# mightypirate1/DRL-Tetris

Measured on AMD Instinct MI355X. Metric: env-steps/sec at 64k parallel 20x10 boards, higher is better.
Workload: dtype u32

## Files before the change

drl-tetris_amd/csrc/tetris_engine.h:

```cpp
#pragma once
#include "tetris_layout.h"
#include "tetris_tables.h"

#if defined(__clang__)
#define TE_UNROLL _Pragma("unroll")
#else
#define TE_UNROLL _Pragma("GCC unroll 8")
#endif

namespace te {

TE_HD int ctz32(uint32_t v) { return __builtin_ctz(v); }
TE_HD int clz32(uint32_t v) { return __builtin_clz(v); }
#if defined(__HIP_DEVICE_COMPILE__)
TE_HD uint32_t ld_stream(const uint32_t* p) { return __builtin_nontemporal_load(p); }
TE_HD void st_stream(uint32_t* p, uint32_t v) { __builtin_nontemporal_store(v, p); }
#else
TE_HD uint32_t ld_stream(const uint32_t* p) { return *p; }
TE_HD void st_stream(uint32_t* p, uint32_t v) { *p = v; }
#endif

#if defined(TE_PATH_COUNTERS) && !defined(__HIPCC__)
enum PathCounter { PC_KICK = 0, PC_KICK_2ND, PC_KICK_3RD, PC_KICK_FAILED, PC_KICK_DOWN, PC_DROP_EXACT, PC_RT_OFF_SPAWN,
                   PC_GARBAGE_ROW, PC_GARBAGE_LIFT2, PC_DEATH_GARBAGE, PC_DEATH_SPAWN, PC_TIMER_LOCK, PC_KEY_KICK, PC_KEY_KICK_FAILED,
// ... 5 lines not shown
#endif

enum MemMode : int { MEM_STREAM = 0, MEM_AGENT = 1, MEM_AFFINE = 2 };
#if defined(__HIP_DEVICE_COMPILE__)
TE_HD uint32_t ld_agent(const uint32_t* p) { return __hip_atomic_load(p, __ATOMIC_RELAXED, __HIP_MEMORY_SCOPE_AGENT); }
TE_HD void st_agent(uint32_t* p, uint32_t v) { __hip_atomic_store(p, v, __ATOMIC_RELAXED, __HIP_MEMORY_SCOPE_AGENT); }
#else
TE_HD uint32_t ld_agent(const uint32_t* p) { return *p; }
TE_HD void st_agent(uint32_t* p, uint32_t v) { *p = v; }
#endif
#if defined(__HIP_DEVICE_COMPILE__)
TE_HD __amdgpu_buffer_rsrc_t te_rsrc(const void* base) {
    return __builtin_amdgcn_make_buffer_rsrc(const_cast<void*>(base), (short)0, -1, 0x00020000);
}
constexpr int TE_AUX_NT = 2, TE_AUX_SC1 = 16;
TE_HD uint32_t ldw_b(const uint32_t* base, uint32_t o, size_t row_bytes, int mem = MEM_STREAM) {
    const __amdgpu_buffer_rsrc_t r = te_rsrc(base);
    if (mem == MEM_AGENT || mem == MEM_AFFINE) return __builtin_amdgcn_raw_buffer_load_b32(r, (int)o, (int)(uint32_t)row_bytes, TE_AUX_SC1);
    return __builtin_amdgcn_raw_buffer_load_b32(r, (int)o, (int)(uint32_t)row_bytes, TE_AUX_NT);
}
TE_HD void stw_b(uint32_t* base, uint32_t o, size_t row_bytes, uint32_t v, int mem = MEM_STREAM) {
    const __amdgpu_buffer_rsrc_t r = te_rsrc(base);
    if (mem == MEM_AGENT) __builtin_amdgcn_raw_buffer_store_b32(v, r, (int)o, (int)(uint32_t)row_bytes, TE_AUX_SC1);
    else if (mem == MEM_AFFINE) __builtin_amdgcn_raw_buffer_store_b32(v, r, (int)o, (int)(uint32_t)row_bytes, 0);
    else __builtin_amdgcn_raw_buffer_store_b32(v, r, (int)o, (int)(uint32_t)row_bytes, TE_AUX_NT);
}
#else
TE_HD uint32_t ldw_b(const uint32_t* base, uint32_t o, size_t row_bytes, int mem = MEM_STREAM) {
    const uint32_t* p = (const uint32_t*)((const char*)base + row_bytes + o);
    return mem != MEM_STREAM ? ld_agent(p) : ld_stream(p);
}
TE_HD void stw_b(uint32_t* base, uint32_t o, size_t row_bytes, uint32_t v, int mem = MEM_STREAM) {
    uint32_t* p = (uint32_t*)((char*)base + row_bytes + o);
    if (mem != MEM_STREAM) st_agent(p, v); else st_stream(p, v);
}
#endif
TE_HD uint32_t ldw(const uint32_t* base, uint32_t o, size_t word_off, int mem = MEM_STREAM) { return ldw_b(base, o, word_off * 4u, mem); }
TE_HD void stw(uint32_t* base, uint32_t o, size_t word_off, uint32_t v, int mem = MEM_STREAM) { stw_b(base, o, word_off * 4u, v, mem); }
struct RowStride { size_t ws; };
template <int N>
struct RowTable { uint32_t bytes[N]; };
TE_HD size_t row_bytes(const RowStride& r, int w) { return (size_t)w * r.ws * 4u; }
template <int N>
TE_HD size_t row_bytes(const RowTable<N>& r, int w) { return r.bytes[w]; }
#if defined(__HIP_DEVICE_COMPILE__)
TE_HD void add_word(uint32_t* p, uint32_t v) { (void)__hip_atomic_fetch_add(p, v, __ATOMIC_RELAXED, __HIP_MEMORY_SCOPE_AGENT); }
#else
TE_HD void add_word(uint32_t* p, uint32_t v) { *p += v; }
#endif
#if defined(__HIP_DEVICE_COMPILE__)
TE_HD uint32_t mul24(uint32_t a, uint32_t b) { return __umul24(a, b); }
#else
TE_HD uint32_t mul24(uint32_t a, uint32_t b) { return a * b; }
#endif
TE_HD int imin(int a, int b) { return a < b ? a : b; }
TE_HD int imax(int a, int b) { return a > b ? a : b; }
TE_HD uint32_t f2u(float f) { union { float f; uint32_t u; } v; v.f = f; return v.u; }
TE_HD float u2f(uint32_t u) { union { float f; uint32_t u; } v; v.u = u; return v.f; }

// ... 86 lines not shown
template <int P>
struct Game {
    Player pl[P];
    uint32_t seed16;
    int round_over, last_winner;
    uint32_t flags;
    uint32_t episode;
    uint32_t steps;
    uint32_t add_lines, add_sent;
    uint32_t status;
    uint32_t draw0, draw1;
};

template <class ROWS>
TE_HD void load_player_rows(const uint32_t* s, uint32_t o, const ROWS& rows, Player& q, bool tint, bool queue = true, int mem = MEM_STREAM) {
    for (int c = 0; c < NCOL; c++) q.col[c] = ldw_b(s, o, row_bytes(rows, W_COL0 + c), mem);
    if (tint)
        for (int k = 0; k < 3; k++)
            for (int c = 0; c < NCOL; c++) q.tint[k][c] = ldw_b(s, o, row_bytes(rows, W_TINT0 + 10 * k + c), mem);
    uint32_t w = ldw_b(s, o, row_bytes(rows, W_PIECE), mem);
    q.kind = w & 7; q.rot = (w >> 3) & 3; q.x = (int)((w >> 5) & 15) - 4; q.y = (w >> 9) & 31;
    q.next = (w >> 14) & 7; q.dead = (w >> 17) & 1; q.lock_armed = (w >> 18) & 1; q.reward = (w >> 19) & 255;
    w = ldw_b(s, o, row_bytes(rows, W_MISC), mem);
    q.inc_count = w & 255; q.combo_count = (w >> 8) & 255; q.line_count = (w >> 16) & 255;
    q.qlen = (w >> 24) & 15; q.q_overflow = (w >> 28) & 3;
    if (!queue) { q.inc_count = 0; q.qlen = 0; q.q_overflow = 0; }
    q.time_ms = (int32_t)ldw_b(s, o, row_bytes(rows, W_TIME), mem);
    w = ldw_b(s, o, row_bytes(rows, W_DROPCOMBO), mem);
    q.drop_delay = w & 0xFFFF; q.combo_remaining = w >> 16;
    q.drop_time = (int32_t)ldw_b(s, o, row_bytes(rows, W_DROP_TIME), mem);
    q.speedup_time = (int32_t)ldw_b(s, o, row_bytes(rows, W_SPEEDUP_TIME), mem);
    q.lock_time = (int32_t)ldw_b(s, o, row_bytes(rows, W_LOCK_TIME), mem);
    q.combo_start = (int32_t)ldw_b(s, o, row_bytes(rows, W_COMBO_START), mem);
    q.combo_time = (int32_t)ldw_b(s, o, row_bytes(rows, W_COMBO_TIME), mem);
    q.incoming = queue ? u2f(ldw_b(s, o, row_bytes(rows, W_INCOMING), mem)) : 0.0f;
    q.min_remaining = queue ? (int32_t)ldw_b(s, o, row_bytes(rows, W_MIN_REMAINING), mem) : 1000;
    q.piece_draws = ldw_b(s, o, row_bytes(rows, W_PIECE_DRAWS), mem);
    q.hole_draws = queue ? ldw_b(s, o, row_bytes(rows, W_HOLE_DRAWS), mem) : 0u;
    q.pgroup = ldw_b(s, o, row_bytes(rows, W_PIECE_GROUP), mem);
    w = ldw_b(s, o, row_bytes(rows, W_STATS0), mem); q.lines_sent = w & 0xFFFF; q.lines_cleared = w >> 16;
    w = ldw_b(s, o, row_bytes(rows, W_STATS1), mem); q.lines_blocked = w & 0xFFFF; q.max_combo = w >> 16;
    w = ldw_b(s, o, row_bytes(rows, W_STATS2), mem); q.lines_seen = w & 0xFFFF; q.garbage_cleared = w >> 16;
    q.q_loaded = queue && q.qlen > 0;
    q.pf_ok = 0; q.pf_raw.lo = 0; q.pf_raw.hi = 0;
    if (queue)
        for (int i = 0; i < FIFO_CAP; i++) { q.qcount[i] = 0; q.qdelay[i] = 0; }
    if (q.q_loaded) {
        for (int i = 0; i < FIFO_CAP / 2; i++) {
            uint32_t cw = ldw_b(s, o, row_bytes(rows, W_FIFO_COUNT0 + i), mem);
            q.qcount[2 * i] = (int16_t)(cw & 0xFFFF);
            q.qcount[2 * i + 1] = (int16_t)(cw >> 16);
        }
        for (int i = 0; i < FIFO_CAP; i++) q.qdelay[i] = (int32_t)ldw_b(s, o, row_bytes(rows, W_FIFO_DELAY0 + i), mem);
    }
}

TE_HD void load_player(const uint32_t* s, uint32_t o, size_t ws, Player& q, bool tint, bool queue = true, int mem = MEM_STREAM) {
    load_player_rows(s, o, RowStride{ws}, q, tint, queue, mem);
}

template <int P, class ROWS>
TE_HD void load_game_words_rows(const Ref& gr, const ROWS& rows, Game<P>& g, bool counters = false, int mem = MEM_STREAM) {
    uint32_t meta = ldw_b(gr.s, gr.o, row_bytes(rows, G_META), mem);
    g.seed16 = meta & 0xFFFFu;
    g.round_over = (meta >> 16) & 1;
    g.last_winner = (int)((meta >> 17) & 0xF) - 1;
    g.flags = (meta >> 21) & 7u;
    g.episode = ldw_b(gr.s, gr.o, row_bytes(rows, G_EPISODE), mem);
    g.steps = counters ? ldw_b(gr.s, gr.o, row_bytes(rows, G_STEPS), mem) : 0u;
    g.add_lines = 0; g.add_sent = 0;
    g.status = 0;
}

template <int P>
TE_HD void load_game_words(const Ref& gr, Game<P>& g, bool counters = false, int mem = MEM_STREAM) {
    load_game_words_rows<P>(gr, RowStride{gr.ws}, g, counters, mem);
}

template <int P, class ROWS, class GROWS>
TE_HD void load_game_rows(const Geo& geo_in, size_t slot, const ROWS& rows, const GROWS& grows, Game<P>& g, bool tint = false, bool queue = true,
                          bool counters = false, int mem = MEM_STREAM) {
    Geo geo = geo_in;
    geo.P = P;
    load_game_words_rows<P>(game_ref(geo, slot), grows, g, counters, mem);
    TE_UNROLL
    for (int p = 0; p < P; p++) {
        const Ref r = board_ref(geo, p, slot);
        load_player_rows(r.s, r.o, rows, g.pl[p], tint, queue, mem);
    }
}
template <int P>
TE_HD void load_game(const Geo& geo_in, size_t slot, Game<P>& g, bool tint = false, bool queue = true, bool counters = false, int mem = MEM_STREAM) {
    load_game_rows<P>(geo_in, slot, RowStride{(size_t)P * geo_in.stride}, RowStride{geo_in.stride}, g, tint, queue, counters, mem);
}

template <class ROWS>
TE_HD void store_player_rows(uint32_t* s, uint32_t o, const ROWS& rows, const Player& q, bool tint, bool queue = true, int mem = MEM_STREAM) {
    for (int c = 0; c < NCOL; c++) stw_b(s, o, row_bytes(rows, W_COL0 + c), q.col[c], mem);
    if (tint)
        for (int k = 0; k < 3; k++)
            for (int c = 0; c < NCOL; c++) stw_b(s, o, row_bytes(rows, W_TINT0 + 10 * k + c), q.tint[k][c], mem);
    stw_b(s, o, row_bytes(rows, W_PIECE), (uint32_t)q.kind | ((uint32_t)q.rot << 3) | ((uint32_t)(q.x + 4) << 5) | ((uint32_t)q.y << 9) |
                              ((uint32_t)q.next << 14) | ((uint32_t)q.dead << 17) | ((uint32_t)q.lock_armed << 18) |
                              ((uint32_t)(q.reward & 255) << 19), mem);
    stw_b(s, o, row_bytes(rows, W_MISC), (uint32_t)(q.inc_count & 255) | ((uint32_t)(q.combo_count & 255) << 8) |
                             ((uint32_t)(q.line_count & 255) << 16) | ((uint32_t)q.qlen << 24) | ((uint32_t)q.q_overflow << 28), mem);
    stw_b(s, o, row_bytes(rows, W_TIME), (uint32_t)q.time_ms, mem);
    stw_b(s, o, row_bytes(rows, W_DROPCOMBO), ((uint32_t)q.drop_delay & 0xFFFF) | (q.combo_remaining << 16), mem);
    stw_b(s, o, row_bytes(rows, W_DROP_TIME), (uint32_t)q.drop_time, mem);
    stw_b(s, o, row_bytes(rows, W_SPEEDUP_TIME), (uint32_t)q.speedup_time, mem);
    stw_b(s, o, row_bytes(rows, W_LOCK_TIME), (uint32_t)q.lock_time, mem);
    stw_b(s, o, row_bytes(rows, W_COMBO_START), (uint32_t)q.combo_start, mem);
    stw_b(s, o, row_bytes(rows, W_COMBO_TIME), (uint32_t)q.combo_time, mem);
    if (queue) stw_b(s, o, row_bytes(rows, W_INCOMING), f2u(q.incoming), mem);
    stw_b(s, o, row_bytes(rows, W_MIN_REMAINING), (uint32_t)q.min_remaining, mem);
    stw_b(s, o, row_bytes(rows, W_PIECE_DRAWS), q.piece_draws, mem);
    if (queue) stw_b(s, o, row_bytes(rows, W_HOLE_DRAWS), q.hole_draws, mem);
    stw_b(s, o, row_bytes(rows, W_PIECE_GROUP), q.pgroup, mem);
    stw_b(s, o, row_bytes(rows, W_STATS0), (q.lines_sent & 0xFFFF) | (q.lines_cleared << 16), mem);
    stw_b(s, o, row_bytes(rows, W_STATS1), (q.lines_blocked & 0xFFFF) | (q.max_combo << 16), mem);
    stw_b(s, o, row_bytes(rows, W_STATS2), (q.lines_seen & 0xFFFF) | (q.garbage_cleared << 16), mem);
    if (queue && (q.q_loaded || q.qlen > 0)) {
        for (int i = 0; i < FIFO_CAP / 2; i++)
            stw_b(s, o, row_bytes(rows, W_FIFO_COUNT0 + i), ((uint32_t)q.qcount[2 * i] & 0xFFFF) | ((uint32_t)q.qcount[2 * i + 1] << 16), mem);
        for (int i = 0; i < FIFO_CAP; i++) stw_b(s, o, row_bytes(rows, W_FIFO_DELAY0 + i), (uint32_t)q.qdelay[i], mem);
    }
}

TE_HD void store_player(uint32_t* s, uint32_t o, size_t ws, const Player& q, bool tint, bool queue = true, int mem = MEM_STREAM) {
    store_player_rows(s, o, RowStride{ws}, q, tint, queue, mem);
}

template <int P, class ROWS>
TE_HD void store_game_words_rows(const Ref& gr, const ROWS& rows, const Game<P>& g, bool counters = false, int mem = MEM_STREAM) {
    stw_b(gr.s, gr.o, row_bytes(rows, G_META), g.seed16 | ((uint32_t)g.round_over << 16) | ((uint32_t)(g.last_winner + 1) << 17) | (g.flags << 21), mem);
    stw_b(gr.s, gr.o, row_bytes(rows, G_EPISODE), g.episode, mem);
    if (counters) stw_b(gr.s, gr.o, row_bytes(rows, G_STEPS), g.steps, mem);
    if (g.add_lines) add_word((uint32_t*)((char*)gr.s + row_bytes(rows, G_LINES) + gr.o), g.add_lines);
    if (g.add_sent) add_word((uint32_t*)((char*)gr.s + row_bytes(rows, G_SENT) + gr.o), g.add_sent);
}

template <int P>
TE_HD void store_game_words(const Ref& gr, const Game<P>& g, bool counters = false, int mem = MEM_STREAM) {
    store_game_words_rows<P>(gr, RowStride{gr.ws}, g, counters, mem);
}

template <int P, class ROWS, class GROWS>
TE_HD void store_game_rows(const Geo& geo_in, size_t slot, const ROWS& rows, const GROWS& grows, const Game<P>& g, bool tint = false, bool queue = true,
                           bool counters = false, int mem = MEM_STREAM) {
    Geo geo = geo_in;
    geo.P = P;
    store_game_words_rows<P>(game_ref(geo, slot), grows, g, counters, mem);
// ... 236 lines not shown
TE_HD int combo_expire(const Ctx& cx, Player& q, int32_t t) {
    int32_t left = q.combo_start + q.combo_time - t;
    q.combo_remaining = left < 0 ? 0u : ((uint32_t)left & 0xFFFFu);
    if (t > q.combo_start + q.combo_time && q.combo_count != 0) {
        float duration = 1.f + (float)t / 60000.f * 0.1f;
        double v = cx.combo_pow[q.combo_count] * (double)duration;
        int lines = (int)((uint32_t)(int64_t)v & 0xFFFFu);
        q.combo_count = 0;
        q.line_count = 0;
        return lines;
    }
    return 0;
}


TE_HD bool spawn_next(const Ctx& cx, Player& q, uint32_t seed16, uint32_t& status) {
    q.kind = q.next;
    q.rot = spawn_rot(q.kind);
    q.x = (NCOL - 4) / 2;
    q.y = 0;
    if (q.piece_draws + cx.margin >= cx.n_draws) {
        status |= ST_NEED_EXTEND;
        if (q.piece_draws >= cx.n_draws) status |= ST_STREAM_EXHAUSTED;
    }
    q.next = (int)((q.pgroup >> (4u * (q.piece_draws & 7u))) & 7u);
    q.piece_draws++;
    if ((q.piece_draws & 7u) == 0u) {
        q.pgroup = pack_group(q.pf_ok ? q.pf_raw : table_group_raw(cx, seed16, q.piece_draws, status));
        q.pf_ok = 0;
    }
    uint32_t shape = shape_of(cx, q.kind, q.rot);
    if (!fits_spawn_col(cx, q, shape, 0)) { stamp(cx, q, shape); TE_COUNT(PC_DEATH_SPAWN); return true; }
    return false;
}

TE_HD int score_clears(const Ctx& cx, Player& q, int cleared) {
    q.lines_cleared = (q.lines_cleared + (uint32_t)cleared) & 0xFFFFu;
    if (cleared == 0) { q.combo_time -= 200; return 0; }
    int amount = cx.queue ? q_block(q, cleared - 1, q.time_ms, true) : cleared - 1;
    q.lines_sent = (q.lines_sent + (uint32_t)amount) & 0xFFFFu;
    combo_gain(q, q.time_ms, cleared);
    return amount;
}

TE_HD void lock_piece(const Ctx& cx, Player& q) {
    uint32_t shape = shape_of(cx, q.kind, q.rot);
    q.y += drop_distance(cx, q, shape);
    stamp(cx, q, shape);
    q.drop_time = q.time_ms;
    q.lock_armed = 0;
}

TE_HD int settle(const Ctx& cx, Player& q, uint32_t seed16, uint32_t& status) {
    int sent = score_clears(cx, q, clear_rows(cx, q));
    if (spawn_next(cx, q, seed16, status)) return -1;
    return sent;
}

TE_HD bool soft_drop(const Ctx& cx, Player& q) {
    const uint32_t shape = shape_of(cx, q.kind, q.rot);
    if (q.x == (NCOL - 4) / 2 ? fits_spawn_col(cx, q, shape, q.y + 1) : fits_at(cx, q, shape, q.x, q.y + 1)) {
        q.y++;
        q.drop_time = q.time_ms;
        q.lock_armed = 0;
        return true;
    }
    if (!q.lock_armed) q.lock_time = q.time_ms + 400;
    q.lock_armed = 1;
    return false;
}
// ... 15 lines not shown
    q.hole_draws++;
    uint32_t bottom = 1u << (cx.H - 1);
    for (int c = 0; c < NCOL; c++) q.col[c] = (q.col[c] >> 1) | (c == hole ? 0u : bottom);
    if (cx.tint)
        for (int k = 0; k < 3; k++)
            for (int c = 0; c < NCOL; c++) q.tint[k][c] = (q.tint[k][c] >> 1) | (c == hole ? 0u : bottom);
    TE_COUNT(PC_GARBAGE_ROW);
    if (q.y > 0) q.y--;
    if (!fits_at(cx, q, shape_of(cx, q.kind, q.rot), q.x, q.y)) {
        if (q.y > 0) { q.y--; TE_COUNT(PC_GARBAGE_LIFT2); }
        else { TE_COUNT(PC_DEATH_GARBAGE); return true; }
    }
    return false;
}

TE_HD int tick(const Ctx& cx, Player& q, int ms, uint32_t seed16, uint32_t& status) {
    q.time_ms += ms;
    if (gravity_due(q, q.time_ms)) soft_drop(cx, q);
    int sent = 0;
    bool finished = false;
    if (q.lock_armed && q.time_ms > q.lock_time && !soft_drop(cx, q)) {
        TE_COUNT(PC_TIMER_LOCK);
        lock_piece(cx, q);
        sent = settle(cx, q, seed16, status);
        finished = true;
    }
    if (!finished) {
        if (cx.queue) {
            int whole = 0;
            while (q.incoming >= 1.0f) { whole++; q.incoming = q.incoming - 1.f; }
            if (whole) q_add(q, whole, q.time_ms, status);
        }
        sent = combo_expire(cx, q, q.time_ms);
        if (sent) {
            if (cx.queue) sent = q_block(q, sent, q.time_ms, false);
            q.lines_sent = (q.lines_sent + (uint32_t)sent) & 0xFFFFu;
        }
        if (cx.queue && q_release(q, q.time_ms))
            if (push_garbage(cx, q, seed16, status)) sent = -1;
// ... 514 lines not shown
    for (int p = 0; p < P; p++)
        if (p != sender) g.pl[p].incoming = g.pl[p].incoming + each;
}

template <int P>
TE_HD bool confine_errors(Game<P>& g) {
    int err = 0;
    TE_UNROLL
    for (int p = 0; p < P; p++) {
        if (g.status & ST_STREAM_EXHAUSTED) g.pl[p].q_overflow |= ERR_STREAM;
        err |= g.pl[p].q_overflow;
    }
    return err != 0;
}

template <int P>
TE_HD int finish_game(const Ctx& cx, Game<P>& g, int ms) {
    if (g.round_over) return 1;
    bool stop = false;
    TE_UNROLL
    for (int p = 0; p < P; p++) {
        Player& q = g.pl[p];
        if (!stop && !q.dead) {
            const int sent = settle(cx, q, g.seed16, g.status);
            if (sent == -1) { q.dead = 1; stop = true; }
            else if (sent) share_lines<P>(g, p, sent);
        }
    }
    int alive = 0;
    TE_UNROLL
    for (int p = 0; p < P; p++) {
        Player& q = g.pl[p];
        if (!q.dead) {
            const int sent = tick(cx, q, ms, g.seed16, g.status);
            if (sent == -1) q.dead = 1;
            else {
                if (sent) share_lines<P>(g, p, sent);
                alive++;
                q.reward = (int)((q.lines_cleared - q.lines_seen) & 0xFFu);
                q.lines_seen = q.lines_cleared;
                q.inc_count = cx.queue ? (q_total(q) & 255) : 0;
            }
        }
    }
    if (confine_errors<P>(g)) { g.round_over = 1; return 1; }
    if ((P > 1 && alive < 2) || !alive) { g.round_over = 1; return 1; }
    return 0;
}

// ... 37 lines not shown
    if (alive < 2 || q.q_overflow || opp_err) { g.round_over = 1; return 1; }
    return 0;
}

TE_HD void reset_split(const Ctx& cx, Game<1>& g, uint32_t seed16) {
    const int side = (int)(g.flags & SPLIT_SIDE);
    const bool me_alive = !g.pl[0].dead, opp_alive = !(g.flags & SPLIT_OPP_DEAD);
    int winner = -1;
    if (me_alive && !opp_alive) winner = side;
    if (opp_alive && !me_alive) winner = 1 - side;
    reset_game<1>(cx, g, seed16);
    g.last_winner = winner;
    g.flags &= ~SPLIT_OPP_DEAD;
}

TE_HD uint32_t episode_seed(uint32_t game, uint32_t episode) { return (12345u + mul24(7919u, game & 0xFFFFu) + mul24(104729u & 0xFFFFu, episode & 0xFFFFu)) & 0xFFFFu; }

TE_HD void philox4x32_10(uint32_t k0, uint32_t c0, uint32_t c1, uint32_t c2, uint32_t out[4]) {
    uint32_t k1 = 0u, c3 = 0u;
    TE_UNROLL
    for (int r = 0; r < 10; r++) {
        uint64_t p0 = (uint64_t)0xD2511F53u * c0;
        uint64_t p1 = (uint64_t)0xCD9E8D57u * c2;
        uint32_t n0 = (uint32_t)(p1 >> 32) ^ c1 ^ k0;
        uint32_t n1 = (uint32_t)p1;
        uint32_t n2 = (uint32_t)(p0 >> 32) ^ c3 ^ k1;
        uint32_t n3 = (uint32_t)p0;
        c0 = n0; c1 = n1; c2 = n2; c3 = n3;
        k0 += 0x9E3779B9u; k1 += 0xBB67AE85u;
    }
    out[0] = c0; out[1] = c1; out[2] = c2; out[3] = c3;
// ... 4 lines not shown
```

drl-tetris_amd/csrc/tetris_hip.hip:

```cpp
#include <hip/hip_runtime.h>
#include <hip/hip_ext.h>

#include <math.h>
#include <stdio.h>
#include <stdlib.h>
#include <string.h>

#include <algorithm>
#include <atomic>
#include <mutex>
#include <thread>
#include <new>
#include <chrono>
#include <string>
#include <vector>

#include "tetris_kernels.h"

using namespace te;


#include "tetris_game_kernel.h"

constexpr int CHAIN_LANES = 64;
// ... 17 lines not shown
        }
        wave = (int)((blockIdx.x & ~7u) | xcc);
        if (wave * CHAIN_LANES >= a.n) { report_xcc(); return; }
    }
    const int i = wave * CHAIN_LANES + lane;
    const bool active = lane < CHAIN_LANES && i < a.n;
    LaneCounters cnt = {0, 0, 0, 0};
    const uint32_t shape_word = d_shape_table.s[lane];
    Game<P> g;
    if (active) policy_draw(a, (uint32_t)i, a.first_step, g.draw0, g.draw1);
    const uint32_t d0 = g.draw0, d1 = g.draw1;
    int stride = a.n_stride;
    asm volatile("" : "+s"(stride));
    RowTable<NWORDS> rows = {};
    RowTable<NGWORDS> grows = {};
    if (!FUSED) {
        TE_UNROLL
        for (int w = 0; w < NWORDS; w++)
            if (P > 1 || (w < NWORDS_HOT && w != W_INCOMING && w != W_HOLE_DRAWS)) {
                uint32_t bytes = (uint32_t)(w * P) * (uint32_t)stride * 4u;
                asm volatile("" : "+s"(bytes));
                rows.bytes[w] = bytes;
            }
        TE_UNROLL
        for (int w = 0; w < NGWORDS; w++) {
            uint32_t bytes = (uint32_t)w * (uint32_t)stride * 4u;
            asm volatile("" : "+s"(bytes));
            grows.bytes[w] = bytes;
        }
    }
    const uint32_t seen = chain_poll(a, (uint32_t)wave);
    if (seen == a.epoch - 1u) {
        Geo geo = geo_of(a);
        geo.stride = (size_t)stride;
        if (active) {
            if (FUSED) load_game<P>(geo, (size_t)i, g, false, P > 1, true, CMEM);
            else load_game_rows<P>(geo, (size_t)i, rows, grows, g, false, P > 1, true, CMEM);
            g.draw0 = d0; g.draw1 = d1;
        }
        s_shapes[lane] = shape_word;
        __builtin_amdgcn_wave_barrier();
        if (FUSED) {
            if (active) game_run<P, M_ROLLOUT, false, CMEM>(a, i, s_shapes, g, cnt);
        } else if (active) {
            const Ctx cx = make_ctx(a, s_shapes, false, P > 1);
            rollout_step<P>(cx, a, (size_t)i, a.first_step, g, cnt);
            store_game_rows<P>(geo, (size_t)i, rows, grows, g, false, P > 1, true, CMEM);
            report_status(a, g.status);
        }
        asm volatile("s_waitcnt vmcnt(0)" ::: "memory");
        if (lane == 0) {
            if (AFFINE) st_xcd(a.chain + (size_t)wave * CHAIN_STRIDE, a.epoch);
            else st_agent(a.chain + (size_t)wave * CHAIN_STRIDE, a.epoch);
        }
    } else if (!(seen & CHAIN_ABANDONED)) {
        chain_give_up(a, (uint32_t)wave, lane == 0);
    }
    report_xcc();
}
template <int P>
__global__ __launch_bounds__(64) void k_chain(KArgs a) { chain_body<P, false, false>(a); }
// ... 2484 lines not shown
```

drl-tetris_amd/csrc/tetris_kernels.h:

```cpp
#pragma once
#include "../../include/tetris_hip.h"
#include "tetris_engine.h"

namespace te {

struct KArgs {
    uint32_t* state;
    uint32_t* gstate;
    uint32_t* status;
    const uint8_t* table;
    const uint64_t* start;
    const double* combo_pow;
    uint32_t n_draws, margin;
    int H;
    int n_games;
    int n_stride;
    int n_players;
    int nw;
    int n;
    const int32_t* idx;
    const uint8_t* keys;
    const uint8_t* lens;
    int max_keys;
    const uint8_t* rot;
// ... 163 lines not shown
TE_HD void policy_draw(const KArgs& a, uint32_t slot, unsigned long long step, uint32_t& w0, uint32_t& w1) {
    uint32_t w[4];
    philox4x32_10(a.policy_seed, a.game_offset + slot, (uint32_t)step, (uint32_t)(step >> 32), w);
    w0 = w[0]; w1 = w[1];
}

template <int P, int MODE, bool TINT = false, int MEM = MEM_STREAM>
TE_HD void game_load(const KArgs& a, int i, Game<P>& g) {
    const size_t slot = a.idx ? (size_t)a.idx[i] : (size_t)i;
    if (MODE != M_INIT && MODE != M_SPLIT_INIT)
        load_game<P>(geo_of(a), slot, g, TINT, P > 1 || MODE == M_SPLIT_RESET, MODE == M_ROLLOUT, MEM);
    if (MODE == M_ROLLOUT) policy_draw(a, (uint32_t)slot, a.first_step, g.draw0, g.draw1);
    if (MODE == M_STEP_RT || MODE == M_STEP_RT_AUTO) { g.draw0 = a.rot[i]; g.draw1 = (uint32_t)a.trans[i] | ((a.player ? (uint32_t)a.player[i] : 0u) << 8); }
}

template <int P>
TE_HD void rollout_step(const Ctx& cx, const KArgs& a, size_t slot, unsigned long long step, Game<P>& g, LaneCounters& cnt) {
    TE_UNROLL
    for (int p = 0; p < P; p++) prefetch_next(cx, g.pl[p], g.seed16, g.status);
    ResetPrefetch rpf;
    prefetch_reset(cx, episode_seed(a.game_offset + (uint32_t)slot, g.episode + 1), rpf);
    int r = (int)(g.draw0 & 3u), t = (int)(g.draw1 % 10u);
    int player = P > 1 ? (int)(step % (unsigned long long)P) : 0;
    uint32_t sent_before = 0;
    TE_UNROLL
    for (int p = 0; p < P; p++) sent_before += g.pl[p].lines_sent;
    make_rt<P>(cx, g, player, r, t);
    int done = finish_game<P>(cx, g, a.ms);
    cnt.steps++;
    g.steps++;
    uint32_t sent_after = 0;
    TE_UNROLL
    for (int p = 0; p < P; p++) {
        sent_after += g.pl[p].lines_sent;
        if (!g.pl[p].dead) { cnt.lines += (unsigned)g.pl[p].reward; g.add_lines += (unsigned)g.pl[p].reward; }
    }
    cnt.sent += (sent_after - sent_before) & 0xFFFFu;
    g.add_sent += (sent_after - sent_before) & 0xFFFFu;
    if (done) {
        cnt.episodes++;
        g.episode++;
        reset_game<P>(cx, g, episode_seed(a.game_offset + (uint32_t)slot, g.episode), &rpf);
    }
}

template <int P, int MODE, bool TINT = false, int MEM = MEM_STREAM>
TE_HD void game_run(const KArgs& a, int i, const uint32_t* shapes, Game<P>& g, LaneCounters& cnt) {
    const size_t slot = a.idx ? (size_t)a.idx[i] : (size_t)i;
    Ctx cx = make_ctx(a, shapes, TINT, P > 1 || MODE == M_SPLIT_INIT || MODE == M_SPLIT_RESET);
    if (MODE == M_INIT) init_game<P>(cx, g, (uint32_t)(a.seeds ? (uint16_t)a.seeds[i] : 0));
    if (MODE == M_SPLIT_INIT) {
        init_game<P>(cx, g, (uint32_t)(a.seeds ? (uint16_t)a.seeds[i] : 0));
        g.flags = SPLIT_ON | (a.steps ? SPLIT_SIDE : 0u);
    } else if (MODE == M_SPLIT_RESET) {
        if (P == 1) reset_split(cx, *reinterpret_cast<Game<1>*>(&g), (uint32_t)(a.seeds ? (uint16_t)a.seeds[i] : 0));
    } else if (MODE == M_RESET) {
        reset_game<P>(cx, g, (uint32_t)(a.seeds ? (uint16_t)a.seeds[i] : 0));
// ... 427 lines not shown
```

Baseline: 22.40 billion.

## Hoist buffer descriptors and lane seed, skip death stamp before reset

Builds the buffer resource descriptors for the state and game-state arrays once and stores them in the row tables, so each load and store no longer rebuilds them. Precomputes the per-lane episode seed, derives two game-word offsets by addition instead of fresh multiplies, and skips stamping the losing piece on spawn death in one-player rollouts, since a reset follows straight away. This aims to cut scalar address setup and wasted work on the death path. The cost is extra template variants and a wider row-table struct that must stay in scalar registers.

New measurement: 22.74 billion, median of 6. 1.5% higher.

```diff
diff --git a/drl-tetris_amd/csrc/tetris_engine.h b/drl-tetris_amd/csrc/tetris_engine.h
--- a/drl-tetris_amd/csrc/tetris_engine.h
+++ b/drl-tetris_amd/csrc/tetris_engine.h
@@ -43,17 +43,17 @@
     return __builtin_amdgcn_make_buffer_rsrc(const_cast<void*>(base), (short)0, -1, 0x00020000);
 }
 constexpr int TE_AUX_NT = 2, TE_AUX_SC1 = 16;
-TE_HD uint32_t ldw_b(const uint32_t* base, uint32_t o, size_t row_bytes, int mem = MEM_STREAM) {
-    const __amdgpu_buffer_rsrc_t r = te_rsrc(base);
+TE_HD uint32_t ldw_r(__amdgpu_buffer_rsrc_t r, uint32_t o, size_t row_bytes, int mem = MEM_STREAM) {
     if (mem == MEM_AGENT || mem == MEM_AFFINE) return __builtin_amdgcn_raw_buffer_load_b32(r, (int)o, (int)(uint32_t)row_bytes, TE_AUX_SC1);
     return __builtin_amdgcn_raw_buffer_load_b32(r, (int)o, (int)(uint32_t)row_bytes, TE_AUX_NT);
 }
-TE_HD void stw_b(uint32_t* base, uint32_t o, size_t row_bytes, uint32_t v, int mem = MEM_STREAM) {
-    const __amdgpu_buffer_rsrc_t r = te_rsrc(base);
+TE_HD void stw_r(__amdgpu_buffer_rsrc_t r, uint32_t o, size_t row_bytes, uint32_t v, int mem = MEM_STREAM) {
     if (mem == MEM_AGENT) __builtin_amdgcn_raw_buffer_store_b32(v, r, (int)o, (int)(uint32_t)row_bytes, TE_AUX_SC1);
     else if (mem == MEM_AFFINE) __builtin_amdgcn_raw_buffer_store_b32(v, r, (int)o, (int)(uint32_t)row_bytes, 0);
     else __builtin_amdgcn_raw_buffer_store_b32(v, r, (int)o, (int)(uint32_t)row_bytes, TE_AUX_NT);
 }
+TE_HD uint32_t ldw_b(const uint32_t* base, uint32_t o, size_t row_bytes, int mem = MEM_STREAM) { return ldw_r(te_rsrc(base), o, row_bytes, mem); }
+TE_HD void stw_b(uint32_t* base, uint32_t o, size_t row_bytes, uint32_t v, int mem = MEM_STREAM) { stw_r(te_rsrc(base), o, row_bytes, v, mem); }
 #else
 TE_HD uint32_t ldw_b(const uint32_t* base, uint32_t o, size_t row_bytes, int mem = MEM_STREAM) {
     const uint32_t* p = (const uint32_t*)((const char*)base + row_bytes + o);
@@ -68,10 +68,25 @@
 TE_HD void stw(uint32_t* base, uint32_t o, size_t word_off, uint32_t v, int mem = MEM_STREAM) { stw_b(base, o, word_off * 4u, v, mem); }
 struct RowStride { size_t ws; };
 template <int N>
-struct RowTable { uint32_t bytes[N]; };
+struct RowTable {
+    uint32_t bytes[N];
+#if defined(__HIP_DEVICE_COMPILE__)
+    __amdgpu_buffer_rsrc_t rsrc;
+#endif
+};
 TE_HD size_t row_bytes(const RowStride& r, int w) { return (size_t)w * r.ws * 4u; }
 template <int N>
 TE_HD size_t row_bytes(const RowTable<N>& r, int w) { return r.bytes[w]; }
+template <class ROWS>
+TE_HD uint32_t ldw_row(const uint32_t* base, uint32_t o, const ROWS& rows, int w, int mem) { return ldw_b(base, o, row_bytes(rows, w), mem); }
+template <class ROWS>
+TE_HD void stw_row(uint32_t* base, uint32_t o, const ROWS& rows, int w, uint32_t v, int mem) { stw_b(base, o, row_bytes(rows, w), v, mem); }
+#if defined(__HIP_DEVICE_COMPILE__)
+template <int N>
+TE_HD uint32_t ldw_row(const uint32_t*, uint32_t o, const RowTable<N>& rows, int w, int mem) { return ldw_r(rows.rsrc, o, rows.bytes[w], mem); }
+template <int N>
+TE_HD void stw_row(uint32_t*, uint32_t o, const RowTable<N>& rows, int w, uint32_t v, int mem) { stw_r(rows.rsrc, o, rows.bytes[w], v, mem); }
+#endif
 #if defined(__HIP_DEVICE_COMPILE__)
 TE_HD void add_word(uint32_t* p, uint32_t v) { (void)__hip_atomic_fetch_add(p, v, __ATOMIC_RELAXED, __HIP_MEMORY_SCOPE_AGENT); }
 #else
@@ -188,44 +203,44 @@
 
 template <class ROWS>
 TE_HD void load_player_rows(const uint32_t* s, uint32_t o, const ROWS& rows, Player& q, bool tint, bool queue = true, int mem = MEM_STREAM) {
-    for (int c = 0; c < NCOL; c++) q.col[c] = ldw_b(s, o, row_bytes(rows, W_COL0 + c), mem);
+    for (int c = 0; c < NCOL; c++) q.col[c] = ldw_row(s, o, rows, W_COL0 + c, mem);
     if (tint)
         for (int k = 0; k < 3; k++)
-            for (int c = 0; c < NCOL; c++) q.tint[k][c] = ldw_b(s, o, row_bytes(rows, W_TINT0 + 10 * k + c), mem);
-    uint32_t w = ldw_b(s, o, row_bytes(rows, W_PIECE), mem);
+            for (int c = 0; c < NCOL; c++) q.tint[k][c] = ldw_row(s, o, rows, W_TINT0 + 10 * k + c, mem);
+    uint32_t w = ldw_row(s, o, rows, W_PIECE, mem);
     q.kind = w & 7; q.rot = (w >> 3) & 3; q.x = (int)((w >> 5) & 15) - 4; q.y = (w >> 9) & 31;
     q.next = (w >> 14) & 7; q.dead = (w >> 17) & 1; q.lock_armed = (w >> 18) & 1; q.reward = (w >> 19) & 255;
-    w = ldw_b(s, o, row_bytes(rows, W_MISC), mem);
+    w = ldw_row(s, o, rows, W_MISC, mem);
     q.inc_count = w & 255; q.combo_count = (w >> 8) & 255; q.line_count = (w >> 16) & 255;
     q.qlen = (w >> 24) & 15; q.q_overflow = (w >> 28) & 3;
     if (!queue) { q.inc_count = 0; q.qlen = 0; q.q_overflow = 0; }
-    q.time_ms = (int32_t)ldw_b(s, o, row_bytes(rows, W_TIME), mem);
-    w = ldw_b(s, o, row_bytes(rows, W_DROPCOMBO), mem);
+    q.time_ms = (int32_t)ldw_row(s, o, rows, W_TIME, mem);
+    w = ldw_row(s, o, rows, W_DROPCOMBO, mem);
     q.drop_delay = w & 0xFFFF; q.combo_remaining = w >> 16;
-    q.drop_time = (int32_t)ldw_b(s, o, row_bytes(rows, W_DROP_TIME), mem);
-    q.speedup_time = (int32_t)ldw_b(s, o, row_bytes(rows, W_SPEEDUP_TIME), mem);
-    q.lock_time = (int32_t)ldw_b(s, o, row_bytes(rows, W_LOCK_TIME), mem);
-    q.combo_start = (int32_t)ldw_b(s, o, row_bytes(rows, W_COMBO_START), mem);
-    q.combo_time = (int32_t)ldw_b(s, o, row_bytes(rows, W_COMBO_TIME), mem);
-    q.incoming = queue ? u2f(ldw_b(s, o, row_bytes(rows, W_INCOMING), mem)) : 0.0f;
-    q.min_remaining = queue ? (int32_t)ldw_b(s, o, row_bytes(rows, W_MIN_REMAINING), mem) : 1000;
-    q.piece_draws = ldw_b(s, o, row_bytes(rows, W_PIECE_DRAWS), mem);
-    q.hole_draws = queue ? ldw_b(s, o, row_bytes(rows, W_HOLE_DRAWS), mem) : 0u;
-    q.pgroup = ldw_b(s, o, row_bytes(rows, W_PIECE_GROUP), mem);
-    w = ldw_b(s, o, row_bytes(rows, W_STATS0), mem); q.lines_sent = w & 0xFFFF; q.lines_cleared = w >> 16;
-    w = ldw_b(s, o, row_bytes(rows, W_STATS1), mem); q.lines_blocked = w & 0xFFFF; q.max_combo = w >> 16;
-    w = ldw_b(s, o, row_bytes(rows, W_STATS2), mem); q.lines_seen = w & 0xFFFF; q.garbage_cleared = w >> 16;
+    q.drop_time = (int32_t)ldw_row(s, o, rows, W_DROP_TIME, mem);
+    q.speedup_time = (int32_t)ldw_row(s, o, rows, W_SPEEDUP_TIME, mem);
+    q.lock_time = (int32_t)ldw_row(s, o, rows, W_LOCK_TIME, mem);
+    q.combo_start = (int32_t)ldw_row(s, o, rows, W_COMBO_START, mem);
+    q.combo_time = (int32_t)ldw_row(s, o, rows, W_COMBO_TIME, mem);
+    q.incoming = queue ? u2f(ldw_row(s, o, rows, W_INCOMING, mem)) : 0.0f;
+    q.min_remaining = queue ? (int32_t)ldw_row(s, o, rows, W_MIN_REMAINING, mem) : 1000;
+    q.piece_draws = ldw_row(s, o, rows, W_PIECE_DRAWS, mem);
+    q.hole_draws = queue ? ldw_row(s, o, rows, W_HOLE_DRAWS, mem) : 0u;
+    q.pgroup = ldw_row(s, o, rows, W_PIECE_GROUP, mem);
+    w = ldw_row(s, o, rows, W_STATS0, mem); q.lines_sent = w & 0xFFFF; q.lines_cleared = w >> 16;
+    w = ldw_row(s, o, rows, W_STATS1, mem); q.lines_blocked = w & 0xFFFF; q.max_combo = w >> 16;
+    w = ldw_row(s, o, rows, W_STATS2, mem); q.lines_seen = w & 0xFFFF; q.garbage_cleared = w >> 16;
     q.q_loaded = queue && q.qlen > 0;
     q.pf_ok = 0; q.pf_raw.lo = 0; q.pf_raw.hi = 0;
     if (queue)
         for (int i = 0; i < FIFO_CAP; i++) { q.qcount[i] = 0; q.qdelay[i] = 0; }
     if (q.q_loaded) {
         for (int i = 0; i < FIFO_CAP / 2; i++) {
-            uint32_t cw = ldw_b(s, o, row_bytes(rows, W_FIFO_COUNT0 + i), mem);
+            uint32_t cw = ldw_row(s, o, rows, W_FIFO_COUNT0 + i, mem);
             q.qcount[2 * i] = (int16_t)(cw & 0xFFFF);
             q.qcount[2 * i + 1] = (int16_t)(cw >> 16);
         }
-        for (int i = 0; i < FIFO_CAP; i++) q.qdelay[i] = (int32_t)ldw_b(s, o, row_bytes(rows, W_FIFO_DELAY0 + i), mem);
+        for (int i = 0; i < FIFO_CAP; i++) q.qdelay[i] = (int32_t)ldw_row(s, o, rows, W_FIFO_DELAY0 + i, mem);
     }
 }
 
@@ -235,13 +250,13 @@
 
 template <int P, class ROWS>
 TE_HD void load_game_words_rows(const Ref& gr, const ROWS& rows, Game<P>& g, bool counters = false, int mem = MEM_STREAM) {
-    uint32_t meta = ldw_b(gr.s, gr.o, row_bytes(rows, G_META), mem);
+    uint32_t meta = ldw_row(gr.s, gr.o, rows, G_META, mem);
     g.seed16 = meta & 0xFFFFu;
     g.round_over = (meta >> 16) & 1;
     g.last_winner = (int)((meta >> 17) & 0xF) - 1;
     g.flags = (meta >> 21) & 7u;
-    g.episode = ldw_b(gr.s, gr.o, row_bytes(rows, G_EPISODE), mem);
-    g.steps = counters ? ldw_b(gr.s, gr.o, row_bytes(rows, G_STEPS), mem) : 0u;
+    g.episode = ldw_row(gr.s, gr.o, rows, G_EPISODE, mem);
+    g.steps = counters ? ldw_row(gr.s, gr.o, rows, G_STEPS, mem) : 0u;
     g.add_lines = 0; g.add_sent = 0;
     g.status = 0;
 }
@@ -270,34 +285,34 @@
 
 template <class ROWS>
 TE_HD void store_player_rows(uint32_t* s, uint32_t o, const ROWS& rows, const Player& q, bool tint, bool queue = true, int mem = MEM_STREAM) {
-    for (int c = 0; c < NCOL; c++) stw_b(s, o, row_bytes(rows, W_COL0 + c), q.col[c], mem);
+    for (int c = 0; c < NCOL; c++) stw_row(s, o, rows, W_COL0 + c, q.col[c], mem);
     if (tint)
         for (int k = 0; k < 3; k++)
-            for (int c = 0; c < NCOL; c++) stw_b(s, o, row_bytes(rows, W_TINT0 + 10 * k + c), q.tint[k][c], mem);
-    stw_b(s, o, row_bytes(rows, W_PIECE), (uint32_t)q.kind | ((uint32_t)q.rot << 3) | ((uint32_t)(q.x + 4) << 5) | ((uint32_t)q.y << 9) |
+            for (int c = 0; c < NCOL; c++) stw_row(s, o, rows, W_TINT0 + 10 * k + c, q.tint[k][c], mem);
+    stw_row(s, o, rows, W_PIECE, (uint32_t)q.kind | ((uint32_t)q.rot << 3) | ((uint32_t)(q.x + 4) << 5) | ((uint32_t)q.y << 9) |
                               ((uint32_t)q.next << 14) | ((uint32_t)q.dead << 17) | ((uint32_t)q.lock_armed << 18) |
                               ((uint32_t)(q.reward & 255) << 19), mem);
-    stw_b(s, o, row_bytes(rows, W_MISC), (uint32_t)(q.inc_count & 255) | ((uint32_t)(q.combo_count & 255) << 8) |
+    stw_row(s, o, rows, W_MISC, (uint32_t)(q.inc_count & 255) | ((uint32_t)(q.combo_count & 255) << 8) |
                              ((uint32_t)(q.line_count & 255) << 16) | ((uint32_t)q.qlen << 24) | ((uint32_t)q.q_overflow << 28), mem);
-    stw_b(s, o, row_bytes(rows, W_TIME), (uint32_t)q.time_ms, mem);
-    stw_b(s, o, row_bytes(rows, W_DROPCOMBO), ((uint32_t)q.drop_delay & 0xFFFF) | (q.combo_remaining << 16), mem);
-    stw_b(s, o, row_bytes(rows, W_DROP_TIME), (uint32_t)q.drop_time, mem);
-    stw_b(s, o, row_bytes(rows, W_SPEEDUP_TIME), (uint32_t)q.speedup_time, mem);
-    stw_b(s, o, row_bytes(rows, W_LOCK_TIME), (uint32_t)q.lock_time, mem);
-    stw_b(s, o, row_bytes(rows, W_COMBO_START), (uint32_t)q.combo_start, mem);
-    stw_b(s, o, row_bytes(rows, W_COMBO_TIME), (uint32_t)q.combo_time, mem);
-    if (queue) stw_b(s, o, row_bytes(rows, W_INCOMING), f2u(q.incoming), mem);
-    stw_b(s, o, row_bytes(rows, W_MIN_REMAINING), (uint32_t)q.min_remaining, mem);
-    stw_b(s, o, row_bytes(rows, W_PIECE_DRAWS), q.piece_draws, mem);
-    if (queue) stw_b(s, o, row_bytes(rows, W_HOLE_DRAWS), q.hole_draws, mem);
-    stw_b(s, o, row_bytes(rows, W_PIECE_GROUP), q.pgroup, mem);
-    stw_b(s, o, row_bytes(rows, W_STATS0), (q.lines_sent & 0xFFFF) | (q.lines_cleared << 16), mem);
-    stw_b(s, o, row_bytes(rows, W_STATS1), (q.lines_blocked & 0xFFFF) | (q.max_combo << 16), mem);
-    stw_b(s, o, row_bytes(rows, W_STATS2), (q.lines_seen & 0xFFFF) | (q.garbage_cleared << 16), mem);
+    stw_row(s, o, rows, W_TIME, (uint32_t)q.time_ms, mem);
+    stw_row(s, o, rows, W_DROPCOMBO, ((uint32_t)q.drop_delay & 0xFFFF) | (q.combo_remaining << 16), mem);
+    stw_row(s, o, rows, W_DROP_TIME, (uint32_t)q.drop_time, mem);
+    stw_row(s, o, rows, W_SPEEDUP_TIME, (uint32_t)q.speedup_time, mem);
+    stw_row(s, o, rows, W_LOCK_TIME, (uint32_t)q.lock_time, mem);
+    stw_row(s, o, rows, W_COMBO_START, (uint32_t)q.combo_start, mem);
+    stw_row(s, o, rows, W_COMBO_TIME, (uint32_t)q.combo_time, mem);
+    if (queue) stw_row(s, o, rows, W_INCOMING, f2u(q.incoming), mem);
+    stw_row(s, o, rows, W_MIN_REMAINING, (uint32_t)q.min_remaining, mem);
+    stw_row(s, o, rows, W_PIECE_DRAWS, q.piece_draws, mem);
+    if (queue) stw_row(s, o, rows, W_HOLE_DRAWS, q.hole_draws, mem);
+    stw_row(s, o, rows, W_PIECE_GROUP, q.pgroup, mem);
+    stw_row(s, o, rows, W_STATS0, (q.lines_sent & 0xFFFF) | (q.lines_cleared << 16), mem);
+    stw_row(s, o, rows, W_STATS1, (q.lines_blocked & 0xFFFF) | (q.max_combo << 16), mem);
+    stw_row(s, o, rows, W_STATS2, (q.lines_seen & 0xFFFF) | (q.garbage_cleared << 16), mem);
     if (queue && (q.q_loaded || q.qlen > 0)) {
         for (int i = 0; i < FIFO_CAP / 2; i++)
-            stw_b(s, o, row_bytes(rows, W_FIFO_COUNT0 + i), ((uint32_t)q.qcount[2 * i] & 0xFFFF) | ((uint32_t)q.qcount[2 * i + 1] << 16), mem);
-        for (int i = 0; i < FIFO_CAP; i++) stw_b(s, o, row_bytes(rows, W_FIFO_DELAY0 + i), (uint32_t)q.qdelay[i], mem);
+            stw_row(s, o, rows, W_FIFO_COUNT0 + i, ((uint32_t)q.qcount[2 * i] & 0xFFFF) | ((uint32_t)q.qcount[2 * i + 1] << 16), mem);
+        for (int i = 0; i < FIFO_CAP; i++) stw_row(s, o, rows, W_FIFO_DELAY0 + i, (uint32_t)q.qdelay[i], mem);
     }
 }
 
@@ -307,9 +322,9 @@
 
 template <int P, class ROWS>
 TE_HD void store_game_words_rows(const Ref& gr, const ROWS& rows, const Game<P>& g, bool counters = false, int mem = MEM_STREAM) {
-    stw_b(gr.s, gr.o, row_bytes(rows, G_META), g.seed16 | ((uint32_t)g.round_over << 16) | ((uint32_t)(g.last_winner + 1) << 17) | (g.flags << 21), mem);
-    stw_b(gr.s, gr.o, row_bytes(rows, G_EPISODE), g.episode, mem);
-    if (counters) stw_b(gr.s, gr.o, row_bytes(rows, G_STEPS), g.steps, mem);
+    stw_row(gr.s, gr.o, rows, G_META, g.seed16 | ((uint32_t)g.round_over << 16) | ((uint32_t)(g.last_winner + 1) << 17) | (g.flags << 21), mem);
+    stw_row(gr.s, gr.o, rows, G_EPISODE, g.episode, mem);
+    if (counters) stw_row(gr.s, gr.o, rows, G_STEPS, g.steps, mem);
     if (g.add_lines) add_word((uint32_t*)((char*)gr.s + row_bytes(rows, G_LINES) + gr.o), g.add_lines);
     if (g.add_sent) add_word((uint32_t*)((char*)gr.s + row_bytes(rows, G_SENT) + gr.o), g.add_sent);
 }
@@ -576,6 +591,7 @@
 }
 
 
+template <bool RESET_FOLLOWS_DEATH = false>
 TE_HD bool spawn_next(const Ctx& cx, Player& q, uint32_t seed16, uint32_t& status) {
     q.kind = q.next;
     q.rot = spawn_rot(q.kind);
@@ -592,7 +608,11 @@
         q.pf_ok = 0;
     }
     uint32_t shape = shape_of(cx, q.kind, q.rot);
-    if (!fits_spawn_col(cx, q, shape, 0)) { stamp(cx, q, shape); TE_COUNT(PC_DEATH_SPAWN); return true; }
+    if (!fits_spawn_col(cx, q, shape, 0)) {
+        if (!RESET_FOLLOWS_DEATH) stamp(cx, q, shape);
+        TE_COUNT(PC_DEATH_SPAWN);
+        return true;
+    }
     return false;
 }
 
@@ -613,9 +633,10 @@
     q.lock_armed = 0;
 }
 
+template <bool RESET_FOLLOWS_DEATH = false>
 TE_HD int settle(const Ctx& cx, Player& q, uint32_t seed16, uint32_t& status) {
     int sent = score_clears(cx, q, clear_rows(cx, q));
-    if (spawn_next(cx, q, seed16, status)) return -1;
+    if (spawn_next<RESET_FOLLOWS_DEATH>(cx, q, seed16, status)) return -1;
     return sent;
 }
 
@@ -661,6 +682,7 @@
     return false;
 }
 
+template <bool RESET_FOLLOWS_DEATH = false>
 TE_HD int tick(const Ctx& cx, Player& q, int ms, uint32_t seed16, uint32_t& status) {
     q.time_ms += ms;
     if (gravity_due(q, q.time_ms)) soft_drop(cx, q);
@@ -669,7 +691,7 @@
     if (q.lock_armed && q.time_ms > q.lock_time && !soft_drop(cx, q)) {
         TE_COUNT(PC_TIMER_LOCK);
         lock_piece(cx, q);
-        sent = settle(cx, q, seed16, status);
+        sent = settle<RESET_FOLLOWS_DEATH>(cx, q, seed16, status);
         finished = true;
     }
     if (!finished) {
@@ -1214,7 +1236,7 @@
     return err != 0;
 }
 
-template <int P>
+template <int P, bool RESET_FOLLOWS_DEATH = false>
 TE_HD int finish_game(const Ctx& cx, Game<P>& g, int ms) {
     if (g.round_over) return 1;
     bool stop = false;
@@ -1222,7 +1244,7 @@
     for (int p = 0; p < P; p++) {
         Player& q = g.pl[p];
         if (!stop && !q.dead) {
-            const int sent = settle(cx, q, g.seed16, g.status);
+            const int sent = settle<RESET_FOLLOWS_DEATH>(cx, q, g.seed16, g.status);
             if (sent == -1) { q.dead = 1; stop = true; }
             else if (sent) share_lines<P>(g, p, sent);
         }
@@ -1232,7 +1254,7 @@
     for (int p = 0; p < P; p++) {
         Player& q = g.pl[p];
         if (!q.dead) {
-            const int sent = tick(cx, q, ms, g.seed16, g.status);
+            const int sent = tick<RESET_FOLLOWS_DEATH>(cx, q, ms, g.seed16, g.status);
             if (sent == -1) q.dead = 1;
             else {
                 if (sent) share_lines<P>(g, p, sent);
@@ -1300,7 +1322,9 @@
     g.flags &= ~SPLIT_OPP_DEAD;
 }
 
-TE_HD uint32_t episode_seed(uint32_t game, uint32_t episode) { return (12345u + mul24(7919u, game & 0xFFFFu) + mul24(104729u & 0xFFFFu, episode & 0xFFFFu)) & 0xFFFFu; }
+TE_HD uint32_t episode_seed_lane(uint32_t game) { return 12345u + mul24(7919u, game & 0xFFFFu); }
+TE_HD uint32_t episode_seed_of(uint32_t lane_seed, uint32_t episode) { return (lane_seed + mul24(104729u & 0xFFFFu, episode & 0xFFFFu)) & 0xFFFFu; }
+TE_HD uint32_t episode_seed(uint32_t game, uint32_t episode) { return episode_seed_of(episode_seed_lane(game), episode); }
 
 TE_HD void philox4x32_10(uint32_t k0, uint32_t c0, uint32_t c1, uint32_t c2, uint32_t out[4]) {
     uint32_t k1 = 0u, c3 = 0u;
diff --git a/drl-tetris_amd/csrc/tetris_hip.hip b/drl-tetris_amd/csrc/tetris_hip.hip
--- a/drl-tetris_amd/csrc/tetris_hip.hip
+++ b/drl-tetris_amd/csrc/tetris_hip.hip
@@ -55,20 +55,30 @@
     asm volatile("" : "+s"(stride));
     RowTable<NWORDS> rows = {};
     RowTable<NGWORDS> grows = {};
+    uint32_t lane_seed = 0;
     if (!FUSED) {
+        lane_seed = episode_seed_lane(a.game_offset + (uint32_t)i);
+#if defined(__HIP_DEVICE_COMPILE__)
+        rows.rsrc = te_rsrc(a.state);
+        grows.rsrc = te_rsrc(a.gstate);
+        asm volatile("" : "+s"(rows.rsrc), "+s"(grows.rsrc), "+v"(lane_seed));
+#endif
         TE_UNROLL
-        for (int w = 0; w < NWORDS; w++)
+        for (int w = 1; w < NWORDS; w++)
             if (P > 1 || (w < NWORDS_HOT && w != W_INCOMING && w != W_HOLE_DRAWS)) {
                 uint32_t bytes = (uint32_t)(w * P) * (uint32_t)stride * 4u;
                 asm volatile("" : "+s"(bytes));
                 rows.bytes[w] = bytes;
             }
         TE_UNROLL
-        for (int w = 0; w < NGWORDS; w++) {
+        for (int w = 1; w < NGWORDS_HOT; w++) {
             uint32_t bytes = (uint32_t)w * (uint32_t)stride * 4u;
             asm volatile("" : "+s"(bytes));
             grows.bytes[w] = bytes;
         }
+        static_assert(G_EPISODE == 1 && G_STEPS == 2 && G_LINES == 3 && G_SENT == 4, "the sums below");
+        grows.bytes[G_LINES] = grows.bytes[G_EPISODE] + grows.bytes[G_STEPS];
+        grows.bytes[G_SENT] = grows.bytes[G_STEPS] + grows.bytes[G_STEPS];
     }
     const uint32_t seen = chain_poll(a, (uint32_t)wave);
     if (seen == a.epoch - 1u) {
@@ -85,7 +95,7 @@
             if (active) game_run<P, M_ROLLOUT, false, CMEM>(a, i, s_shapes, g, cnt);
         } else if (active) {
             const Ctx cx = make_ctx(a, s_shapes, false, P > 1);
-            rollout_step<P>(cx, a, (size_t)i, a.first_step, g, cnt);
+            rollout_step<P, true>(cx, a, (size_t)i, a.first_step, g, cnt, lane_seed);
             store_game_rows<P>(geo, (size_t)i, rows, grows, g, false, P > 1, true, CMEM);
             report_status(a, g.status);
         }
diff --git a/drl-tetris_amd/csrc/tetris_kernels.h b/drl-tetris_amd/csrc/tetris_kernels.h
--- a/drl-tetris_amd/csrc/tetris_kernels.h
+++ b/drl-tetris_amd/csrc/tetris_kernels.h
@@ -201,19 +201,19 @@
     if (MODE == M_STEP_RT || MODE == M_STEP_RT_AUTO) { g.draw0 = a.rot[i]; g.draw1 = (uint32_t)a.trans[i] | ((a.player ? (uint32_t)a.player[i] : 0u) << 8); }
 }
 
-template <int P>
-TE_HD void rollout_step(const Ctx& cx, const KArgs& a, size_t slot, unsigned long long step, Game<P>& g, LaneCounters& cnt) {
+template <int P, bool HAVE_LANE_SEED = false>
+TE_HD void rollout_step(const Ctx& cx, const KArgs& a, size_t slot, unsigned long long step, Game<P>& g, LaneCounters& cnt, uint32_t lane_seed = 0) {
     TE_UNROLL
     for (int p = 0; p < P; p++) prefetch_next(cx, g.pl[p], g.seed16, g.status);
     ResetPrefetch rpf;
-    prefetch_reset(cx, episode_seed(a.game_offset + (uint32_t)slot, g.episode + 1), rpf);
+    prefetch_reset(cx, HAVE_LANE_SEED ? episode_seed_of(lane_seed, g.episode + 1) : episode_seed(a.game_offset + (uint32_t)slot, g.episode + 1), rpf);
     int r = (int)(g.draw0 & 3u), t = (int)(g.draw1 % 10u);
     int player = P > 1 ? (int)(step % (unsigned long long)P) : 0;
     uint32_t sent_before = 0;
     TE_UNROLL
     for (int p = 0; p < P; p++) sent_before += g.pl[p].lines_sent;
     make_rt<P>(cx, g, player, r, t);
-    int done = finish_game<P>(cx, g, a.ms);
+    int done = finish_game<P, P == 1>(cx, g, a.ms);
     cnt.steps++;
     g.steps++;
     uint32_t sent_after = 0;
@@ -227,7 +227,7 @@
     if (done) {
         cnt.episodes++;
         g.episode++;
-        reset_game<P>(cx, g, episode_seed(a.game_offset + (uint32_t)slot, g.episode), &rpf);
+        reset_game<P>(cx, g, HAVE_LANE_SEED ? episode_seed_of(lane_seed, g.episode) : episode_seed(a.game_offset + (uint32_t)slot, g.episode), &rpf);
     }
 }
 
diff --git a/profiles/isa_compare.py b/profiles/isa_compare.py
--- /dev/null
+++ b/profiles/isa_compare.py
@@ -0,0 +1,65 @@
+import os
+import re
+import shutil
+import subprocess
+import sys
+import tempfile
+
+
+def _tool(name):
+    for cand in (os.path.join(os.environ.get("ROCM_PATH", "/opt/rocm"), "llvm", "bin", name), shutil.which(name)):
+        if cand and os.path.exists(cand):
+            return cand
+    sys.exit(f"{name} not found")
+
+
+def kernels(lib):
+    objdump = _tool("llvm-objdump")
+    out = {}
+    with tempfile.TemporaryDirectory() as d:
+        shutil.copy(lib, os.path.join(d, "lib.so"))
+        subprocess.run([objdump, "--offloading", "lib.so"], cwd=d, check=True, capture_output=True)
+        for f in sorted(os.listdir(d)):
+            if "gfx950" not in f:
+                continue
+            text = subprocess.run([objdump, "-d", "--demangle", "--no-show-raw-insn", "--no-leading-addr", os.path.join(d, f)],
+                                  capture_output=True, text=True, check=True).stdout
+            name = None
+            for line in text.splitlines():
+                m = re.match(r"^(?:[0-9a-f]+ )?<(.*)>:$", line)
+                if m:
+                    name = m.group(1)
+                    out.setdefault(name, [])
+                elif name and line[:1] in ("\t", " ") and line.strip():
+                    out[name].append(line.partition("//")[0].strip())
+    return out
+
+
+def masked(ins):
+    res, n, k = list(ins), 0, 0
+    while k < len(res):
+        if res[k].startswith("s_getpc_b64"):
+            for j in (k + 1, k + 2):
+                if j < len(res) and re.match(r"s_addc?_u32 ", res[j]):
+                    new = re.sub(r"(0x[0-9a-f]+|-?\d+)$", "LIT", res[j])
+                    n += new != res[j]
+                    res[j] = new
+        k += 1
+    return res, n
+
+
+def main(before, after):
+    a, b = kernels(before), kernels(after)
+    print(f"# kernels: {len(a)} before, {len(b)} after; only before: {sorted(set(a) - set(b)) or 'none'}; only after: {sorted(set(b) - set(a)) or 'none'}")
+    for name in sorted(set(a) & set(b)):
+        x, y = a[name], b[name]
+        if x == y:
+            verdict = "identical"
+        else:
+            (mx, nx), (my, _) = masked(x), masked(y)
+            verdict = f"identical but for {nx} pc-relative literals" if mx == my else "DIFFERENT"
+        print(f"{len(x):6d} {len(y):6d}  {verdict:44s}  {name}")
+
+
+if __name__ == "__main__":
+    main(sys.argv[1], sys.argv[2])
diff --git a/profiles/path_census.py b/profiles/path_census.py
--- /dev/null
+++ b/profiles/path_census.py
@@ -0,0 +1,53 @@
+import os
+import sys
+
+ROOT = os.path.dirname(os.path.dirname(os.path.abspath(__file__)))
+sys.path.insert(0, ROOT)
+os.environ.setdefault("OMP_NUM_THREADS", "1")
+
+import __graft_entry__ as ge
+from tests import engines
+
+SEED, MS, LANES, BATCHES, WARM, STEADY = 3441, 400, 64, 128, 64, 128
+
+
+def census():
+    pkg = ge.package()
+    lane = {"fresh": dict.fromkeys(engines.PATH_COUNTERS, 0), "steady": dict.fromkeys(engines.PATH_COUNTERS, 0)}
+    wave = {"fresh": dict.fromkeys(engines.PATH_COUNTERS, 0), "steady": dict.fromkeys(engines.PATH_COUNTERS, 0)}
+    steps = {"fresh": 0, "steady": 0}
+    for b in range(BATCHES):
+        eng = pkg.TetrisBatch(LANES, 1, 20, 10, lib_path=ge.build_harness())
+        eng.set_game_offset(b * LANES)
+        engines.harness_path_counts()
+        for s in range(WARM + STEADY):
+            eng.rollout_random(1, 1, policy_seed=SEED, first_step=s, ms=MS)
+            regime = "fresh" if s < WARM else "steady"
+            steps[regime] += 1
+            for k, v in engines.harness_path_counts().items():
+                lane[regime][k] += v
+                wave[regime][k] += v > 0
+        eng.close()
+    return lane, wave, steps
+
+
+def main():
+    lane, wave, steps = census()
+    out = os.path.join(ROOT, "profiles", "death_path", "path_census.txt")
+    os.makedirs(os.path.dirname(out), exist_ok=True)
+    with open(out, "w") as f:
+        f.write(f"# profiles/path_census.py: {BATCHES} batches of {LANES} one-player games (20 x 10) on the CPU harness, one step per call, policy seed {SEED},\n"
+                f"# {MS} ms; fresh = steps 0..{WARM - 1} from new boards, steady = steps {WARM}..{WARM + STEADY - 1}.  per lane = count / (games x steps);\n"
+                "# per wave = share of (batch, step) pairs in which the counter moved, i.e. in which a wave of these 64 games runs the path;\n"
+                "# 1-(1-p)^64 = what the per-lane rate would give for independent lanes, for comparison.\n")
+        for regime in ("fresh", "steady"):
+            f.write(f"\n{regime}: {steps[regime]} wave-steps, {steps[regime] * LANES} lane-steps\n")
+            f.write(f"{'path':18s} {'per lane':>10s} {'per wave':>10s} {'1-(1-p)^64':>11s}\n")
+            for k in engines.PATH_COUNTERS:
+                p = lane[regime][k] / (steps[regime] * LANES)
+                f.write(f"{k:18s} {p:10.4f} {wave[regime][k] / steps[regime]:10.4f} {1 - (1 - p) ** LANES:11.4f}\n")
+    print(open(out).read())
+
+
+if __name__ == "__main__":
+    main()
```
